# VIS4ROB-lab/covins

Hardware: AMD Instinct MI355X
Metric: GBA iterations/sec, 5-agent EuRoC merged map (higher is better)
Workload: dtype f64

## Files before the change

### covins_amd/csrc/common.hpp

```cpp
#pragma once
#include <hip/hip_runtime.h>
#include <atomic>
#include <cstdlib>
#include <stdint.h>

#include <map>
#include <unordered_map>
#include <utility>
#include <vector>

#include "../../include/covgpu.h"

namespace covgpu {

constexpr int kTile = 128;

struct DevProblem {
  int K, A, L, O, I, E, S;
  int D;
  int n;
  int npad;
  int N;
  int vi;
  int lm_group;
// ... 26 lines not shown
  double *pre_delta;
  double *pre_J;
  double *pre_P;
  double *pre_W;
  double *pre_bias;

  int *edge_i, *edge_j;
  double *edge_meas, *edge_sqrt_info, *edge_loss_a;

  int nchains;
  int max_chain_len;
  int* perm;
  int* pos_kf;
  int* chain_ptr;
  int* pos_chain_end;

  double* Sred;
  double* bred;
  double *Ad, *Ae;
  double *Bp, *Bs, *Bn;
  int* pos_chain_begin;
  double* bp;
  double* grad;
  double* hdiag;
  double* HllInv;
  double* gn;
  double* step;
  double* vtmp;
  double* Linv;
  double* scal;
  double* part;
  int part_n, part_imu, part_edge, part_vec;
  double *imuAd, *imuBs, *imuCd, *imuG;
  double* edgeOut;
  int *kf_edge_ptr, *kf_edge_ent;
  int nepairs;
  int *epair_ptr, *epair_i, *epair_j, *epair_ent;
  int* flag;

  int shard;
  double* vw;

  int nd, nd_nnodes, nd_nlev, nd_maxd;
  int *nd_vnode, *nd_voff, *nd_vord;
  int *nd_vown;
  int *nd_ndepth, *nd_nI;
  long long* nd_ntab;
  int* nd_abase;
  int* nd_fidx;
  double *nd_M, *nd_rhs, *nd_Linv;
  double* nd_dummy;

  double* tr;
  double* scal_r; int* flag_r;

  int uni;
  int* cam_model;
  double* cam_xi;
};

enum {
  TR_RADIUS = 0, TR_MU, TR_LMDF, TR_COST, TR_ALPHA, TR_GG, TR_GN2, TR_GDOT, TR_DNORM, TR_CG, TR_CN, TR_MODEL, TR_SN, TR_RHO, TR_COSTNEW,
  TR_OK, TR_VALID, TR_ACC, TR_TERM, TR_FNCONV, TR_RETRY, TR_FIRST, TR_INITCOST, TR_REUSE,
  TR_JA, TR_JB, TR_JC, TR_VV, TR_VG, TR_NN, TR_XN2,
  TR_COUNT = 32
};
// ... 396 lines not shown
```

### covins_amd/csrc/k_inertial.hip

```cpp
#include "common.hpp"
#include "dev_math.hpp"
#include "reduce.hpp"
#include "inertial_dev.hpp"

namespace covgpu {
using namespace covdev;

__global__ __launch_bounds__(64 * kImuWaves) void k_preintegrate(DevProblem P) {
  __shared__ double sm[kImuWaves][225 * 4 + 270];
  const int lane = threadIdx.x & 63, wave = threadIdx.x >> 6;
  const int f = blockIdx.x * kImuWaves + wave;
  const bool live = f < P.I;
  double* F = sm[wave];
  double* J = F + 225;
  double* C = J + 225;
  double* T = C + 225;
  double* V = T + 225;
  const int fj = live ? P.imu_j[f] : 0;
  const V3 ba = ld3(P.sb + 9 * fj + 3), bg = ld3(P.sb + 9 * fj + 6);
  for (int k = lane; k < 225; k += 64) { F[k] = 0.0; J[k] = (k % 16 == 0) ? 1.0 : 0.0; C[k] = 0.0; }
  for (int k = lane; k < 270; k += 64) V[k] = 0.0;
  V3 dp = v3(0, 0, 0), dv = v3(0, 0, 0);
  Q4 dq = Q4{0, 0, 0, 1};
  double dtsum = 0.0;
  V3 a0 = live ? ld3(P.imu_first + 6 * (size_t)f) : v3(0, 0, 0), w0 = live ? ld3(P.imu_first + 6 * (size_t)f + 3) : v3(0, 0, 0);
  const double* nz = P.imu_noise + 5 * (size_t)(live ? f : 0);
  const double sa = nz[0], sg = nz[1], saw = nz[2], sgw = nz[3];
  const double nd[6] = {sa * sa, sg * sg, sa * sa, sg * sg, saw * saw, sgw * sgw};
  const M3 I3 = ident3();
  __shared__ int s_steps[kImuWaves];
  if (lane == 0) s_steps[wave] = live ? P.imu_ptr[f + 1] - P.imu_ptr[f] : 0;
  __syncthreads();
  int nmax = 0;
#pragma unroll
  for (int k = 0; k < kImuWaves; ++k) nmax = max(nmax, s_steps[k]);
  const int s0 = live ? P.imu_ptr[f] : 0, ns = s_steps[wave];
  for (int it = 0; it < nmax; ++it) {
    const bool on = it < ns;
    if (on && lane == 0) {
      const double* smp = P.imu_samples + 7 * (size_t)(s0 + it);
      const double dt = smp[0];
      const V3 a1 = ld3(smp + 1), w1 = ld3(smp + 4);
      const V3 w = (w0 + w1) * 0.5 - bg;
      const Q4 dq1 = qnormalize(qmul(dq, Q4{w.x * dt * 0.5, w.y * dt * 0.5, w.z * dt * 0.5, 1.0}));
      const M3 Rq = qrot(dq), Rr = qrot(dq1);
      const V3 abar = (mul(Rq, a0 - ba) + mul(Rr, a1 - ba)) * 0.5;
      const V3 dp1 = dp + dv * dt + abar * (0.5 * dt * dt);
      const V3 dv1 = dv + abar * dt;
      const M3 RqA0 = mul(Rq, skew(a0 - ba)), RrA1 = mul(Rr, skew(a1 - ba));
      const M3 ImO = add(I3, scaled(skew(w), -dt));
      const M3 RrA1ImO = mul(RrA1, ImO);
      const M3 RqRr = add(Rq, Rr);
      const double dt2 = dt * dt, dt3 = dt2 * dt;
      set3(F, 15, 0, 0, I3, 1.0);
      set3(F, 15, 0, 3, add(scaled(RqA0, -0.25 * dt2), scaled(RrA1ImO, -0.25 * dt2)), 1.0);
      set3(F, 15, 0, 6, I3, dt);
      set3(F, 15, 0, 9, RqRr, -0.25 * dt2);
      set3(F, 15, 0, 12, RrA1, 0.25 * dt3);
      set3(F, 15, 3, 3, ImO, 1.0);
      set3(F, 15, 3, 12, I3, -dt);
      set3(F, 15, 6, 3, add(scaled(RqA0, -0.5 * dt), scaled(RrA1ImO, -0.5 * dt)), 1.0);
      set3(F, 15, 6, 6, I3, 1.0);
      set3(F, 15, 6, 9, RqRr, -0.5 * dt);
      set3(F, 15, 6, 12, RrA1, 0.5 * dt2);
      set3(F, 15, 9, 9, I3, 1.0);
      set3(F, 15, 12, 12, I3, 1.0);
      set3(V, 18, 0, 0, Rq, 0.25 * dt2);
      set3(V, 18, 0, 3, RrA1, -0.125 * dt3);
      set3(V, 18, 0, 6, Rr, 0.25 * dt2);
      set3(V, 18, 0, 9, RrA1, -0.125 * dt3);
      set3(V, 18, 3, 3, I3, 0.5 * dt);
      set3(V, 18, 3, 9, I3, 0.5 * dt);
      set3(V, 18, 6, 0, Rq, 0.5 * dt);
      set3(V, 18, 6, 3, RrA1, -0.25 * dt2);
      set3(V, 18, 6, 6, Rr, 0.5 * dt);
      set3(V, 18, 6, 9, RrA1, -0.25 * dt2);
      set3(V, 18, 9, 12, I3, dt);
      set3(V, 18, 12, 15, I3, dt);
      dp = dp1; dv = dv1; dq = dq1; dtsum += dt;
      a0 = a1; w0 = w1;
    }
    __syncthreads();
    double jn[4], tn[4];
    if (on) {
#pragma unroll
      for (int u = 0; u < 4; ++u) {
        const int e = lane + 64 * u;
        if (e < 225) {
          const int r = e / 15, c = e - 15 * r;
          double s2 = 0.0, s3 = 0.0;
#pragma unroll
          for (int k = 0; k < 15; ++k) { s2 += F[15 * r + k] * J[15 * k + c]; s3 += F[15 * r + k] * C[15 * k + c]; }
          jn[u] = s2; tn[u] = s3;
        }
      }
    }
    __syncthreads();
    if (on) {
#pragma unroll
      for (int u = 0; u < 4; ++u) {
        const int e = lane + 64 * u;
        if (e < 225) { J[e] = jn[u]; T[e] = tn[u]; }
      }
    }
    __syncthreads();
    if (on) {
#pragma unroll
      for (int u = 0; u < 4; ++u) {
        const int e = lane + 64 * u;
        if (e < 225) {
          const int r = e / 15, c = e - 15 * r;
          double s2 = 0.0;
#pragma unroll
          for (int k = 0; k < 15; ++k) s2 += T[15 * r + k] * F[15 * c + k];
#pragma unroll
          for (int k = 0; k < 18; ++k) s2 += V[18 * r + k] * nd[k / 3] * V[18 * c + k];
          C[e] = s2;
        }
      }
    }
    __syncthreads();
  }
  if (!live) return;
  if (lane == 0) {
    double* d = P.pre_delta + 11 * (size_t)f;
    d[0] = dp.x; d[1] = dp.y; d[2] = dp.z; d[3] = dq.x; d[4] = dq.y; d[5] = dq.z; d[6] = dq.w;
    d[7] = dv.x; d[8] = dv.y; d[9] = dv.z; d[10] = dtsum;
    double* pb = P.pre_bias + 6 * (size_t)f;
    pb[0] = ba.x; pb[1] = ba.y; pb[2] = ba.z; pb[3] = bg.x; pb[4] = bg.y; pb[5] = bg.z;
  }
  for (int k = lane; k < 225; k += 64) { P.pre_J[225 * (size_t)f + k] = J[k]; P.pre_P[225 * (size_t)f + k] = C[k]; }
  __builtin_amdgcn_fence(__ATOMIC_ACQ_REL, "workgroup");
  __builtin_amdgcn_wave_barrier();
  double* Wm = P.pre_W + 225 * (size_t)f;
  if (lane == 0) {
    bool ok = true;
    for (int c = 0; c < 15 && ok; ++c) {
      double dd = C[16 * c];
      for (int k = 0; k < c; ++k) dd -= C[15 * c + k] * C[15 * c + k];
      if (!(dd > 0.0)) { ok = false; break; }
      dd = sqrt(dd);
      C[16 * c] = dd;
      for (int r = c + 1; r < 15; ++r) {
        double s2 = C[15 * r + c];
        for (int k = 0; k < c; ++k) s2 -= C[15 * r + k] * C[15 * c + k];
        C[15 * r + c] = s2 / dd;
      }
    }
    for (int k = 0; k < 225; ++k) F[k] = 0.0;
    if (!ok) atomicAdd(P.flag + 1, 1);
    if (ok)
      for (int c = 0; c < 15; ++c) {
        F[16 * c] = 1.0 / C[16 * c];
        for (int r = c + 1; r < 15; ++r) {
          double s2 = 0.0;
          for (int k = c; k < r; ++k) s2 += C[15 * r + k] * F[15 * k + c];
          F[15 * r + c] = -s2 / C[16 * r];
        }
      }
    for (int k = 0; k < 225; ++k) Wm[k] = F[k];
  }
}

__global__ __launch_bounds__(64 * kImuWaves) void k_imu_build(DevProblem P) {
  __shared__ double sm[kImuWaves][kImuLds];
  const int lane = threadIdx.x & 63, wave = threadIdx.x >> 6;
  const int f = blockIdx.x * kImuWaves + wave;
  const bool live = f < P.I;
  double* sl = sm[wave];
  imu_stage<true>(P, P.pose, P.sb, f, live, lane, sl);
  {
    double c2 = (live && lane < 15) ? 0.5 * sl[1141 + lane] * sl[1141 + lane] : 0.0;
    c2 = wave_sum(c2);
    part_put(P, SC_COST, P.part_imu + blockIdx.x * kImuWaves + wave, c2);
  }
  if (!live) return;
  const double* Jw = sl + 450;
  const double* r = sl + 1141;
  const int i = P.imu_i[f], j = P.imu_j[f];
  const int pi = P.perm[i], pj = P.perm[j];
  const size_t K = (size_t)P.K;
  if (lane < 30) {
    const int a = lane, role = a / 15, la = a % 15;
    double ga = 0.0, haa = 0.0;
    for (int k = 0; k < 15; ++k) { ga += Jw[30 * k + a] * r[k]; haa += Jw[30 * k + a] * Jw[30 * k + a]; }
    double* g = P.imuG + (role * K + (role ? pj : pi)) * 30;
    g[la] = ga; g[15 + la] = haa;
  }
  for (int e = lane; e < 900; e += 64) {
    const int a = e / 30, b = e - 30 * a;
    const int ga_ = a / 15, la = a % 15, gb_ = b / 15, lb = b % 15;
    double h = 0.0;
#pragma unroll
    for (int k = 0; k < 15; ++k) h += Jw[30 * k + a] * Jw[30 * k + b];
    const size_t slot = ga_ * K + (ga_ ? pj : pi);
    if (la < 6 && lb < 6) {
      if (ga_ == gb_) P.imuCd[slot * 36 + 6 * la + lb] = h;
      else if (ga_ == 1) P.imuCd[(2 * K + pj) * 36 + 6 * la + lb] = h;
    } else if (la >= 6 && lb >= 6) {
      if (ga_ == gb_) P.imuAd[slot * 81 + 9 * (la - 6) + (lb - 6)] = h;
      else if (ga_ == 1) P.Ae[(size_t)81 * pj + 9 * (la - 6) + (lb - 6)] = h;
    } else if (la >= 6) {
      if (ga_ == gb_) P.imuBs[slot * 54 + 6 * (la - 6) + lb] = h;
      else if (ga_ == 0) P.Bn[(size_t)54 * pi + 6 * (la - 6) + lb] = h;
      else P.Bp[(size_t)54 * pj + 6 * (la - 6) + lb] = h;
    }
  }
}

__global__ __launch_bounds__(256) void k_imu_gather(DevProblem P, int which) {
  const int t = blockIdx.x * blockDim.x + threadIdx.x;
// ... 99 lines not shown
```

### covins_amd/csrc/k_tail.hip

```cpp
#include "between_dev.hpp"
#include "common.hpp"
#include "dev_math.hpp"
#include "inertial_dev.hpp"
#include "reduce.hpp"
#include "visual_dev.hpp"

namespace covgpu {
using namespace covdev;

static inline int tail_grid(int n, int cap) {
  const int b = (n + 255) / 256;
  return b < 1 ? 1 : (b > cap ? cap : b);
}
COV_DEV void tail_put(const DevProblem& P, double v, int slot, int index) {
  v = wave_sum(v);
  part_put(P, slot, index, v);
}

__global__ __launch_bounds__(256) void k_tail_stats(DevProblem P) {
  double gg = 0, gn2 = 0, gd = 0, gm = 0, vv = 0, vg = 0, nn = 0, xn = 0;
  const int stride = gridDim.x * blockDim.x, t0 = blockIdx.x * blockDim.x + threadIdx.x;
  for (int q = t0; q < P.N; q += stride) {
    const double g = P.grad[q], d = clamp_diag(P.hdiag[q]), s = P.gn[q];
    const double w = P.vw ? P.vw[q] : 1.0;
    const double c = g / (d * d);
    P.vtmp[q] = c;
    gg += w * (g / d) * (g / d); gn2 += w * (d * s) * (d * s); gd += w * g * s; gm = fmax(gm, w * fabs(g));
    vv += w * c * c; vg += w * c * s; nn += w * s * s;
  }
  for (int t = t0; t < P.K; t += stride) {
    const double wp = P.vw ? P.vw[(size_t)P.D * t] : 1.0, ws = (P.vw && P.vi) ? P.vw[(size_t)P.D * t + 6] : 1.0;
    if (!P.fixed[t]) for (int k = 0; k < 7; ++k) xn += wp * P.pose[7 * t + k] * P.pose[7 * t + k];
    if (P.vi) for (int k = 0; k < 9; ++k) xn += ws * P.sb[9 * t + k] * P.sb[9 * t + k];
  }
  for (int q = t0; q < 3 * P.L; q += stride) xn += P.lm[q] * P.lm[q];
  const int idx = P.part_vec + blockIdx.x * 4 + (threadIdx.x >> 6);
  tail_put(P, gg, SC_GG, idx); tail_put(P, gn2, SC_GN2, idx); tail_put(P, gd, SC_GDOT, idx);
  tail_put(P, vv, SC_VV, idx); tail_put(P, vg, SC_VG, idx); tail_put(P, nn, SC_NN, idx); tail_put(P, xn, SC_XN2, idx);
#pragma unroll
  for (int off = 32; off >= 1; off >>= 1) gm = fmax(gm, __shfl_xor(gm, off, 64));
  if ((threadIdx.x & 63) == 0) atomicMax(reinterpret_cast<unsigned long long*>(&P.scal[SC_GMAX]), (unsigned long long)__double_as_longlong(gm));
}

static_assert(kImuWaves == 4, "k_tail_jvp / k_tail_cost index their IMU and edge segments as 4 waves / 256 threads per workgroup");
template <bool TWO, bool UNI>
__global__ __launch_bounds__(64 * kImuWaves) void k_tail_jvp(DevProblem P, const double* __restrict__ va, const double* __restrict__ vb, int nb_obs, int nb_imu) {
  __shared__ double sm[kImuWaves][kImuLds];
  const int lane = threadIdx.x & 63, wave = threadIdx.x >> 6;
  double ja = 0.0, jb = 0.0, jc = 0.0;
  int idx;
  if ((int)blockIdx.x < nb_obs) {
    for (int o = blockIdx.x * blockDim.x + threadIdx.x; o < P.O; o += nb_obs * blockDim.x) {
      ObsLin e;
      const int kf = P.obs_kf[o], l = P.obs_lm[o];
      eval_obs<true, UNI>(P, P.pose, P.lm, o, kf, l, e);
      {
        const double* vp = vb + (size_t)P.D * kf;
        const double* vl = vb + P.n + 3 * (size_t)l;
        double s0 = e.jl[0] * vl[0] + e.jl[1] * vl[1] + e.jl[2] * vl[2];
        double s1 = e.jl[3] * vl[0] + e.jl[4] * vl[1] + e.jl[5] * vl[2];
#pragma unroll
        for (int k = 0; k < 6; ++k) { s0 += e.jp[k] * vp[k]; s1 += e.jp[6 + k] * vp[k]; }
        jb += s0 * s0 + s1 * s1;
        if (TWO) {
          const double* up = va + (size_t)P.D * kf;
          const double* ul = va + P.n + 3 * (size_t)l;
          double t0 = e.jl[0] * ul[0] + e.jl[1] * ul[1] + e.jl[2] * ul[2];
          double t1 = e.jl[3] * ul[0] + e.jl[4] * ul[1] + e.jl[5] * ul[2];
#pragma unroll
          for (int k = 0; k < 6; ++k) { t0 += e.jp[k] * up[k]; t1 += e.jp[6 + k] * up[k]; }
          ja += t0 * t0 + t1 * t1; jc += t0 * s0 + t1 * s1;
        }
      }
    }
    idx = blockIdx.x * 4 + wave;
  } else if ((int)blockIdx.x < nb_obs + nb_imu) {
    const int bi = blockIdx.x - nb_obs;
    const int f = bi * kImuWaves + wave;
    const bool live = f < P.I;
    double* sl = sm[wave];
    imu_stage<true>(P, P.pose, P.sb, f, live, lane, sl);
    if (live && lane < 15) {
      const double* Jw = sl + 450;
      const size_t oi = 15 * (size_t)P.imu_i[f], oj = 15 * (size_t)P.imu_j[f];
      double s2 = 0.0, t2 = 0.0;
      for (int c = 0; c < 15; ++c) {
        s2 += Jw[30 * lane + c] * vb[oi + c] + Jw[30 * lane + 15 + c] * vb[oj + c];
        if (TWO) t2 += Jw[30 * lane + c] * va[oi + c] + Jw[30 * lane + 15 + c] * va[oj + c];
      }
      jb = s2 * s2; ja = t2 * t2; jc = s2 * t2;
    }
    idx = P.part_imu + bi * kImuWaves + wave;
  } else {
    const int be = blockIdx.x - nb_obs - nb_imu;
    const int e = be * 256 + threadIdx.x;
    if (e < P.E) {
      double r[6], J[72];
      eval_edge<true>(P, P.pose, e, r, J);
      const size_t oi = (size_t)P.D * P.edge_i[e], oj = (size_t)P.D * P.edge_j[e];
#pragma unroll
      for (int a = 0; a < 6; ++a) {
        double s = 0.0, t = 0.0;
#pragma unroll
        for (int c = 0; c < 6; ++c) {
          s += J[12 * a + c] * vb[oi + c] + J[12 * a + 6 + c] * vb[oj + c];
          if (TWO) t += J[12 * a + c] * va[oi + c] + J[12 * a + 6 + c] * va[oj + c];
        }
        jb += s * s; ja += t * t; jc += s * t;
      }
    }
    idx = P.part_edge + be * 4 + wave;
    if (be * 4 + wave >= (P.E + 63) / 64) idx = -1;
  }
  jb = wave_sum(jb);
  if (TWO) { ja = wave_sum(ja); jc = wave_sum(jc); }
  if (idx >= 0) {
    part_put(P, SC_JB, idx, jb);
    if (TWO) { part_put(P, SC_JA, idx, ja); part_put(P, SC_JC, idx, jc); }
  }
}

template <bool UNI>
// ... 143 lines not shown
  if (stage == 1) tail_logic_a(P, tc, fresh, rd, P.flag_r[0]);
  else tail_logic_b(P, tc, rd);
}

__global__ __launch_bounds__(256) void k_tail_apply(DevProblem P) {
  const double cg = P.tr[TR_CG], cn = P.tr[TR_CN];
  const int t = blockIdx.x * blockDim.x + threadIdx.x;
  auto st = [&](size_t q) { const double s = cn * P.gn[q]; return cg != 0.0 ? s + cg * P.vtmp[q] : s; };
  if (t < P.K) {
    const size_t b = (size_t)P.D * t;
    const double* x = P.pose + 7 * t;
    double* y = P.pose_c + 7 * t;
    if (P.fixed[t]) {
      for (int k = 0; k < 7; ++k) y[k] = x[k];
    } else {
      const Q4 q = qnormalize(qmul(ldq(x), qexp(V3{st(b), st(b + 1), st(b + 2)})));
      y[0] = q.x; y[1] = q.y; y[2] = q.z; y[3] = q.w;
      y[4] = x[4] + st(b + 3); y[5] = x[5] + st(b + 4); y[6] = x[6] + st(b + 5);
    }
    if (P.vi)
      for (int k = 0; k < 9; ++k) P.sb_c[9 * t + k] = P.sb[9 * t + k] + st(b + 6 + k);
  }
  for (int q = t; q < 3 * P.L; q += gridDim.x * blockDim.x) P.lm_c[q] = P.lm[q] + st((size_t)P.n + q);
}

static inline void tail_segments(const DevProblem& P, int& nb_obs, int& nb_imu, int& nb_edge) {
  nb_obs = P.O > 0 ? tail_grid(P.O, 2048) : 0;
  nb_imu = (P.vi && P.I > 0) ? (P.I + kImuWaves - 1) / kImuWaves : 0;
  nb_edge = P.E > 0 ? (P.E + 255) / 256 : 0;
}
void launch_tail_stats(const DevProblem& P, hipStream_t st) {
  hipLaunchKernelGGL(k_tail_stats, dim3(tail_grid(P.N, 256)), dim3(256), 0, st, P);
}
void launch_tail_jvp(const DevProblem& P, bool two, hipStream_t st) {
  int a, b, c;
  tail_segments(P, a, b, c);
  if (a + b + c == 0) return;
  if (P.uni) {
    if (two) hipLaunchKernelGGL((k_tail_jvp<true, true>), dim3(a + b + c), dim3(64 * kImuWaves), 0, st, P, (const double*)P.vtmp, (const double*)P.gn, a, b);
    else hipLaunchKernelGGL((k_tail_jvp<false, true>), dim3(a + b + c), dim3(64 * kImuWaves), 0, st, P, (const double*)nullptr, (const double*)P.gn, a, b);
    return;
  }
  if (two) hipLaunchKernelGGL((k_tail_jvp<true, false>), dim3(a + b + c), dim3(64 * kImuWaves), 0, st, P, (const double*)P.vtmp, (const double*)P.gn, a, b);
  else hipLaunchKernelGGL((k_tail_jvp<false, false>), dim3(a + b + c), dim3(64 * kImuWaves), 0, st, P, (const double*)nullptr, (const double*)P.gn, a, b);
}
void launch_tail_cost(const DevProblem& P, hipStream_t st) {
  int a, b, c;
  tail_segments(P, a, b, c);
  if (a + b + c == 0) return;
  if (P.uni) hipLaunchKernelGGL(k_tail_cost<true>, dim3(a + b + c), dim3(64 * kImuWaves), 0, st, P, a, b);
  else hipLaunchKernelGGL(k_tail_cost<false>, dim3(a + b + c), dim3(64 * kImuWaves), 0, st, P, a, b);
}
void launch_tail_finish(const DevProblem& P, TrConsts tc, int stage, bool two, bool with_logic, int fresh, hipStream_t st) {
  SlotList sl;
  sl.n = 0;
  auto add = [&](int s) { sl.slot[sl.n++] = s; };
  if (stage == 1) {
    add(SC_GG); add(SC_GN2); add(SC_GDOT); add(SC_VV); add(SC_VG); add(SC_NN); add(SC_XN2); add(SC_JB);
    if (two) { add(SC_JA); add(SC_JC); }
  } else add(SC_COST);
  for (int i = sl.n; i < 12; ++i) sl.slot[i] = 0;
  hipLaunchKernelGGL(k_tail_finish, dim3(sl.n), dim3(1024), 0, st, P, sl, tc, with_logic ? stage : 0, fresh);
}
void launch_tail_logic(const DevProblem& P, TrConsts tc, int stage, int fresh, hipStream_t st) {
  hipLaunchKernelGGL(k_tail_logic, dim3(1), dim3(64), 0, st, P, tc, stage, fresh);
}
void launch_tail_apply(const DevProblem& P, hipStream_t st) {
  const int n = P.K > 3 * P.L ? P.K : 3 * P.L;
  int g = (P.K + 255) / 256;
  const int g2 = tail_grid(n, 2048);
  if (g2 > g) g = g2;
  hipLaunchKernelGGL(k_tail_apply, dim3(g), dim3(256), 0, st, P);
}

}
```

### covins_amd/csrc/solver.hip

```cpp
#include <dlfcn.h>

#include <algorithm>
#include <atomic>
#include <chrono>
#include <condition_variable>
#include <memory>
#include <mutex>
#include <cmath>
#include <cstdio>
#include <cstdlib>
#include <cstring>
#include <string>
#include <thread>
#include <vector>

#include "common.hpp"
#include "nd_plan.hpp"

using namespace covgpu;

static thread_local std::string g_err;
extern "C" const char* covgpu_last_error(void) { return g_err.c_str(); }

#define HIPCHK(expr)                                                                            \
// ... 812 lines not shown
  RC(dev_upload(c, &P.edge_i, (const int*)p->edge_i, (size_t)P.E));
  RC(dev_upload(c, &P.edge_j, (const int*)p->edge_j, (size_t)P.E));
  RC(dev_upload(c, &P.edge_meas, p->edge_meas, (size_t)7 * P.E));
  RC(dev_upload(c, &P.edge_sqrt_info, p->edge_sqrt_info, (size_t)36 * P.E));
  RC(dev_upload(c, &P.edge_loss_a, p->edge_loss_a, (size_t)P.E));
  RC(dev_upload(c, &P.perm, perm.data(), K)); RC(dev_upload(c, &P.pos_kf, pos_kf.data(), K));
  RC(dev_upload(c, &P.chain_ptr, chain_ptr.data(), chain_ptr.size()));
  RC(dev_upload(c, &P.pos_chain_end, chain_end.data(), K));
  RC(dev_alloc(c, &P.bred, (size_t)P.n));
  RC(dev_alloc(c, &P.bp, (size_t)2 * P.npad));
  const size_t Kv = vi ? K : 0;
  RC(dev_alloc(c, &P.Ad, 81 * Kv)); RC(dev_alloc(c, &P.Ae, 81 * Kv));
  RC(dev_alloc(c, &P.Bp, 54 * Kv)); RC(dev_alloc(c, &P.Bs, 54 * Kv)); RC(dev_alloc(c, &P.Bn, 54 * Kv));
  {
    std::vector<int> cbeg(P.K);
    for (int ch = 0; ch < P.nchains; ++ch) for (int q = chain_ptr[ch]; q < chain_ptr[ch + 1]; ++q) cbeg[q] = chain_ptr[ch];
    RC(dev_upload(c, &P.pos_chain_begin, cbeg.data(), cbeg.size()));
    HIPCHK(hipStreamSynchronize(c->st));
  }
  RC(dev_alloc(c, &P.grad, (size_t)P.N)); RC(dev_alloc(c, &P.hdiag, (size_t)P.N));
  RC(dev_alloc(c, &P.HllInv, (size_t)6 * P.L));
  RC(dev_alloc(c, &P.gn, (size_t)P.N)); RC(dev_alloc(c, &P.step, (size_t)P.N)); RC(dev_alloc(c, &P.vtmp, (size_t)P.N));
  HIPCHK(hipMemsetAsync(P.gn, 0, (size_t)P.N * sizeof(double), c->st)); HIPCHK(hipMemsetAsync(P.step, 0, (size_t)P.N * sizeof(double), c->st));
  HIPCHK(hipMemsetAsync(P.vtmp, 0, (size_t)P.N * sizeof(double), c->st));
  RC(dev_alloc(c, &P.scal, (size_t)SC_COUNT)); RC(dev_alloc(c, &P.flag, (size_t)4));
  RC(dev_alloc(c, &P.tr, (size_t)TR_COUNT));
  P.scal_r = P.scal; P.flag_r = P.flag;
  P.part_imu = 8192; P.part_edge = P.part_imu + ((P.I + 3) / 4) * 4; P.part_vec = P.part_edge + (P.E + 63) / 64;
  P.part_n = P.part_vec + 8192;
  RC(dev_alloc(c, &P.part, (size_t)SC_COUNT * P.part_n));
  HIPCHK(hipMemsetAsync(P.part, 0, (size_t)SC_COUNT * P.part_n * sizeof(double), c->st));
  RC(dev_alloc(c, &P.imuAd, 2 * 81 * Kv)); RC(dev_alloc(c, &P.imuBs, 2 * 54 * Kv));
  RC(dev_alloc(c, &P.imuCd, 3 * 36 * Kv)); RC(dev_alloc(c, &P.imuG, 2 * 30 * Kv));
  RC(dev_alloc(c, &P.edgeOut, (size_t)132 * P.E));
  {
    std::vector<int> kptr(P.K + 1, 0), kent(2 * (size_t)P.E);
    for (int e = 0; e < P.E; ++e) {
      if (p->edge_i[e] == p->edge_j[e]) { g_err = "invalid problem: self edge"; return COVGPU_ERR_INVALID_ARG; }
      kptr[p->edge_i[e] + 1]++; kptr[p->edge_j[e] + 1]++;
    }
    for (int k = 0; k < P.K; ++k) kptr[k + 1] += kptr[k];
    { std::vector<int> cur(kptr.begin(), kptr.end() - 1);
      for (int e = 0; e < P.E; ++e) { kent[cur[p->edge_i[e]]++] = 2 * e; kent[cur[p->edge_j[e]]++] = 2 * e + 1; } }
    struct PE { int i, j, ent; };
    std::vector<PE> pe(P.E);
    for (int e = 0; e < P.E; ++e) {
      const int a = perm[p->edge_i[e]], b = perm[p->edge_j[e]];
      pe[e] = (a > b) ? PE{a, b, 2 * e} : PE{b, a, 2 * e + 1};
    }
    std::stable_sort(pe.begin(), pe.end(), [](const PE& x, const PE& y) { return x.i != y.i ? x.i < y.i : x.j < y.j; });
    std::vector<int> eptr, ei, ej, eent(P.E);
    for (int q = 0; q < P.E; ++q) {
      if (q == 0 || pe[q].i != pe[q - 1].i || pe[q].j != pe[q - 1].j) { eptr.push_back(q); ei.push_back(pe[q].i); ej.push_back(pe[q].j); }
      eent[q] = pe[q].ent;
    }
    eptr.push_back(P.E);
    P.nepairs = (int)ei.size();
    RC(dev_upload(c, &P.kf_edge_ptr, kptr.data(), kptr.size())); RC(dev_upload(c, &P.kf_edge_ent, kent.data(), kent.size()));
    RC(dev_upload(c, &P.epair_ptr, eptr.data(), eptr.size())); RC(dev_upload(c, &P.epair_i, ei.data(), ei.size()));
    RC(dev_upload(c, &P.epair_j, ej.data(), ej.size())); RC(dev_upload(c, &P.epair_ent, eent.data(), eent.size()));
    HIPCHK(hipStreamSynchronize(c->st));
    tm("IMU, edges, vectors");
    if (use_nd) {
      NdHostPlan nhp;
      if (c->sharded) {
        if ((int)c->shard_plan->K != P.K || (c->shard_plan->vi != 0) != vi) { g_err = "sharded solve: the problem does not match the shard plan"; return COVGPU_ERR_INVALID_ARG; }
// ... 279 lines not shown
        if (why) { if (!c->coll_failed) { c->coll_failed = true; c->coll_err = why; } c->reducer->abort(); break; }
      } else if (spins > 256) std::this_thread::sleep_for(std::chrono::microseconds(50));
    }
  }
  HIPCHK(hipStreamSynchronize(c->st));
  HIPCHK(hipGetLastError());
  if (dist_sharded(c) && (c->coll_failed || c->chol.gate_failed())) return dist_fail(c);
  if (c->chol.gate_failed()) {
    g_err = "solve: a device-flag gate between the context's streams timed out (COVGPU_GATE_TIMEOUT_S; COVGPU_GATES=0 selects HIP events)";
    return COVGPU_ERR_GATE_TIMEOUT;
  }
  if (c->coll_failed) {
    if (c->reducer) c->reducer->abort();
    if (c->peer_fail) c->peer_fail->store(1);
    g_err = (c->sharded ? "sharded solve, rank " + std::to_string(c->rank) + ": " : std::string("solve: ")) + c->coll_err;
    return COVGPU_ERR_NO_DEVICE;
  }
  return COVGPU_OK;
}

static int solve_impl_dev(covgpu_context* c, const covgpu_options* opt, covgpu_result* res) {
  if (!c->have) { g_err = "no problem uploaded"; return COVGPU_ERR_INVALID_ARG; }
  HIPCHK(hipSetDevice(c->device));
  DevProblem& P = c->P;
  const covgpu_options& o = *opt;
  P.reproj_loss_a = o.reproj_loss_a;
  std::memset(res, 0, sizeof(*res));
  c->coll_failed = false; c->coll_err.clear();
  const auto t_begin = std::chrono::steady_clock::now();
  c->chol.init();
  if (c->sharded) c->chol.gate_timeout_s = std::max(c->chol.gate_timeout_s, 120.0);
  RC(reset_state(c));
  HIPCHK(hipMemsetAsync(P.flag + 1, 0, sizeof(int), c->st));
  launch_preintegrate(P, c->st);
  double* h = c->h_tr;
  std::memset(h, 0, TR_COUNT * sizeof(double));
  h[TR_RADIUS] = o.initial_radius; h[TR_MU] = 1e-8; h[TR_LMDF] = 2.0; h[TR_FIRST] = 1.0; h[TR_OK] = 1.0;
  HIPCHK(hipMemcpyAsync(P.tr, h, TR_COUNT * sizeof(double), hipMemcpyHostToDevice, c->st));
  HIPCHK(hipStreamSynchronize(c->st));
  const TrConsts tc{o.strategy, o.max_radius, o.min_relative_decrease, o.function_tolerance, o.parameter_tolerance, o.gradient_tolerance};
  bool reuse = false, got_initial = false;
  int it = 0, accepted = 0, term = 0;
  static const bool fused_tail = env_int("COVGPU_TAIL", 1) != 0;
  const bool two = o.strategy == COVGPU_DOGLEG;
  const bool coll = c->sharded && c->reducer != nullptr;
  bool use_box = false;
  while (it < o.max_iterations) {
    use_box = false;
    if (fused_tail) {
      if (!reuse) {
        const double damp = (o.strategy == COVGPU_LM) ? 1.0 / h[TR_RADIUS] : h[TR_MU];
        enqueue_build(c, damp);
        enqueue_solve(c, P.gn);
        launch_tail_stats(P, c->st);
        launch_tail_jvp(P, two, c->st);
        launch_tail_finish(P, tc, 1, two, !coll, 1, c->st);
        if (coll) { reduce_scalars(c); launch_tail_logic(P, tc, 1, 1, c->st); }
      } else launch_tail_logic(P, tc, 1, 0, c->st);
      launch_tail_apply(P, c->st);
      launch_tail_cost(P, c->st);
      launch_tail_finish(P, tc, 2, two, !coll, 0, c->st);
      if (coll) { reduce_scalars(c); launch_tail_logic(P, tc, 2, 0, c->st); }
      static const bool dev_aids = getenv("COVGPU_TRACE_PANELS") != nullptr || getenv("COVGPU_GATE_LOG") != nullptr;
      use_box = c->d_box != nullptr && !coll && !c->profiling && !dev_aids;
      if (use_box) c->box_seq += 1.0;
      launch_tr_accept(P, c->st, use_box ? c->d_box : nullptr, c->box_seq);
    } else {
    if (!reuse) {
      const double damp = (o.strategy == COVGPU_LM) ? 1.0 / h[TR_RADIUS] : h[TR_MU];
      enqueue_build(c, damp);
      enqueue_solve(c, P.gn);
      if (o.strategy == COVGPU_DOGLEG) { launch_cauchy_vec(P, c->st); enqueue_jvp(c, P.vtmp); }
// ... 1314 lines not shown
```

Before: 291.2.

## Cache IMU whitened Jacobians for tail JVP and restructure preintegration kernel

The IMU build kernel now stores each factor's whitened Jacobian in a new device buffer (imuJw). The tail JVP kernel reads that buffer instead of re-running imu_stage every iteration; the old path stays behind the COVGPU_IMU_JW env switch. Preintegration is rewritten to exploit the sparsity of F and V with compact 11- and 12-column layouts, to use wave-level syncs instead of block-wide ones, to prefetch the next IMU sample, and to run the Cholesky and inverse across lanes instead of lane 0 alone. Preintegration is also launched on a different stream (chol.mid) after the host sync, which relies on some ordering against the later build kernels that is not visible here. The cache costs extra memory traffic and 450 doubles of storage per factor.

Result: faster. 297.5 (median of 6 runs) (+2.2%).

```diff
diff --git a/covins_amd/csrc/common.hpp b/covins_amd/csrc/common.hpp
--- a/covins_amd/csrc/common.hpp
+++ b/covins_amd/csrc/common.hpp
@@ -82,6 +82,7 @@
   double* part;
   int part_n, part_imu, part_edge, part_vec;
   double *imuAd, *imuBs, *imuCd, *imuG;
+  double* imuJw;
   double* edgeOut;
   int *kf_edge_ptr, *kf_edge_ent;
   int nepairs;
diff --git a/covins_amd/csrc/k_inertial.hip b/covins_amd/csrc/k_inertial.hip
--- a/covins_amd/csrc/k_inertial.hip
+++ b/covins_amd/csrc/k_inertial.hip
@@ -6,122 +6,162 @@
 namespace covgpu {
 using namespace covdev;
 
+COV_DEV void wave_sync() {
+  __builtin_amdgcn_fence(__ATOMIC_ACQ_REL, "workgroup");
+  __builtin_amdgcn_wave_barrier();
+}
+COV_DEV int f_col(int r, int t) {
+  if (r < 3) return t == 0 ? r : t < 4 ? 2 + t : t == 4 ? 6 + r : 4 + t;
+  if (r < 6) return t < 3 ? 3 + t : t == 3 ? 9 + r : 0;
+  if (r < 9) return t < 3 ? 3 + t : t == 3 ? r : t < 10 ? 5 + t : 0;
+  return t == 0 ? r : 0;
+}
+COV_DEV unsigned long long f_cols(int r) {
+  unsigned long long p = 0;
+#pragma unroll
+  for (int t = 0; t < 11; ++t) p |= (unsigned long long)f_col(r, t) << (4 * t);
+  return p;
+}
+constexpr int kPreLds = 225 + 225 + 135 + 165 + 108 + 1;
+static_assert(135 + 165 >= 225, "the whitening matrix is inverted in the slice of T and Fs");
+
 __global__ __launch_bounds__(64 * kImuWaves) void k_preintegrate(DevProblem P) {
-  __shared__ double sm[kImuWaves][225 * 4 + 270];
-  const int lane = threadIdx.x & 63, wave = threadIdx.x >> 6;
-  const int f = blockIdx.x * kImuWaves + wave;
-  const bool live = f < P.I;
-  double* F = sm[wave];
-  double* J = F + 225;
+  __shared__ double sm[kImuWaves][kPreLds];
+  const int lane = threadIdx.x & 63, wave = threadIdx.x >> 6;
+  const int f = blockIdx.x * kImuWaves + wave;
+  if (f >= P.I) return;
+  double* J = sm[wave];
   double* C = J + 225;
   double* T = C + 225;
-  double* V = T + 225;
-  const int fj = live ? P.imu_j[f] : 0;
+  double* Fs = T + 135;
+  double* Vs = Fs + 165;
+  double* sdt = Vs + 108;
+  const int fj = P.imu_j[f];
   const V3 ba = ld3(P.sb + 9 * fj + 3), bg = ld3(P.sb + 9 * fj + 6);
-  for (int k = lane; k < 225; k += 64) { F[k] = 0.0; J[k] = (k % 16 == 0) ? 1.0 : 0.0; C[k] = 0.0; }
-  for (int k = lane; k < 270; k += 64) V[k] = 0.0;
+  for (int k = lane; k < 225; k += 64) { J[k] = (k % 16 == 0) ? 1.0 : 0.0; C[k] = 0.0; }
+  for (int k = lane; k < 165; k += 64) {
+    const int r = k / 11, t = k - 11 * r;
+    Fs[k] = ((r < 3 || r >= 9) ? t == 0 : (r >= 6 && t == 3)) ? 1.0 : 0.0;
+  }
+  for (int k = lane; k < 108; k += 64) Vs[k] = 0.0;
   V3 dp = v3(0, 0, 0), dv = v3(0, 0, 0);
   Q4 dq = Q4{0, 0, 0, 1};
   double dtsum = 0.0;
-  V3 a0 = live ? ld3(P.imu_first + 6 * (size_t)f) : v3(0, 0, 0), w0 = live ? ld3(P.imu_first + 6 * (size_t)f + 3) : v3(0, 0, 0);
-  const double* nz = P.imu_noise + 5 * (size_t)(live ? f : 0);
+  V3 a0 = ld3(P.imu_first + 6 * (size_t)f), w0 = ld3(P.imu_first + 6 * (size_t)f + 3);
+  const double* nz = P.imu_noise + 5 * (size_t)f;
   const double sa = nz[0], sg = nz[1], saw = nz[2], sgw = nz[3];
   const double nd[6] = {sa * sa, sg * sg, sa * sa, sg * sg, saw * saw, sgw * sgw};
   const M3 I3 = ident3();
-  __shared__ int s_steps[kImuWaves];
-  if (lane == 0) s_steps[wave] = live ? P.imu_ptr[f + 1] - P.imu_ptr[f] : 0;
-  __syncthreads();
-  int nmax = 0;
-#pragma unroll
-  for (int k = 0; k < kImuWaves; ++k) nmax = max(nmax, s_steps[k]);
-  const int s0 = live ? P.imu_ptr[f] : 0, ns = s_steps[wave];
-  for (int it = 0; it < nmax; ++it) {
-    const bool on = it < ns;
-    if (on && lane == 0) {
-      const double* smp = P.imu_samples + 7 * (size_t)(s0 + it);
+  const int s0 = P.imu_ptr[f], ns = P.imu_ptr[f + 1] - s0;
+  M3 Rq = qrot(dq), RqA0 = mul(Rq, skew(a0 - ba));
+  V3 Rqa0 = mul(Rq, a0 - ba);
+  unsigned long long pr[3], pc[4];
+#pragma unroll
+  for (int u = 0; u < 3; ++u) pr[u] = f_cols(min((lane + 64 * u) / 15, 14));
+#pragma unroll
+  for (int u = 0; u < 4; ++u) pc[u] = f_cols(min(lane + 64 * u, 224) % 15);
+  double smp[7];
+  if (lane == 0 && ns > 0) {
+#pragma unroll
+    for (int k = 0; k < 7; ++k) smp[k] = P.imu_samples[7 * (size_t)s0 + k];
+  }
+  wave_sync();
+  for (int it = 0; it < ns; ++it) {
+    if (lane == 0) {
       const double dt = smp[0];
-      const V3 a1 = ld3(smp + 1), w1 = ld3(smp + 4);
+      const V3 a1 = v3(smp[1], smp[2], smp[3]), w1 = v3(smp[4], smp[5], smp[6]);
+      if (it + 1 < ns) {
+#pragma unroll
+        for (int k = 0; k < 7; ++k) smp[k] = P.imu_samples[7 * (size_t)(s0 + it + 1) + k];
+      }
       const V3 w = (w0 + w1) * 0.5 - bg;
       const Q4 dq1 = qnormalize(qmul(dq, Q4{w.x * dt * 0.5, w.y * dt * 0.5, w.z * dt * 0.5, 1.0}));
-      const M3 Rq = qrot(dq), Rr = qrot(dq1);
-      const V3 abar = (mul(Rq, a0 - ba) + mul(Rr, a1 - ba)) * 0.5;
+      const M3 Rr = qrot(dq1);
+      const V3 Rra1 = mul(Rr, a1 - ba);
+      const V3 abar = (Rqa0 + Rra1) * 0.5;
       const V3 dp1 = dp + dv * dt + abar * (0.5 * dt * dt);
       const V3 dv1 = dv + abar * dt;
-      const M3 RqA0 = mul(Rq, skew(a0 - ba)), RrA1 = mul(Rr, skew(a1 - ba));
+      const M3 RrA1 = mul(Rr, skew(a1 - ba));
       const M3 ImO = add(I3, scaled(skew(w), -dt));
       const M3 RrA1ImO = mul(RrA1, ImO);
       const M3 RqRr = add(Rq, Rr);
       const double dt2 = dt * dt, dt3 = dt2 * dt;
-      set3(F, 15, 0, 0, I3, 1.0);
-      set3(F, 15, 0, 3, add(scaled(RqA0, -0.25 * dt2), scaled(RrA1ImO, -0.25 * dt2)), 1.0);
-      set3(F, 15, 0, 6, I3, dt);
-      set3(F, 15, 0, 9, RqRr, -0.25 * dt2);
-      set3(F, 15, 0, 12, RrA1, 0.25 * dt3);
-      set3(F, 15, 3, 3, ImO, 1.0);
-      set3(F, 15, 3, 12, I3, -dt);
-      set3(F, 15, 6, 3, add(scaled(RqA0, -0.5 * dt), scaled(RrA1ImO, -0.5 * dt)), 1.0);
-      set3(F, 15, 6, 6, I3, 1.0);
-      set3(F, 15, 6, 9, RqRr, -0.5 * dt);
-      set3(F, 15, 6, 12, RrA1, 0.5 * dt2);
-      set3(F, 15, 9, 9, I3, 1.0);
-      set3(F, 15, 12, 12, I3, 1.0);
-      set3(V, 18, 0, 0, Rq, 0.25 * dt2);
-      set3(V, 18, 0, 3, RrA1, -0.125 * dt3);
-      set3(V, 18, 0, 6, Rr, 0.25 * dt2);
-      set3(V, 18, 0, 9, RrA1, -0.125 * dt3);
-      set3(V, 18, 3, 3, I3, 0.5 * dt);
-      set3(V, 18, 3, 9, I3, 0.5 * dt);
-      set3(V, 18, 6, 0, Rq, 0.5 * dt);
-      set3(V, 18, 6, 3, RrA1, -0.25 * dt2);
-      set3(V, 18, 6, 6, Rr, 0.5 * dt);
-      set3(V, 18, 6, 9, RrA1, -0.25 * dt2);
-      set3(V, 18, 9, 12, I3, dt);
-      set3(V, 18, 12, 15, I3, dt);
+      set3(Fs, 11, 0, 1, add(scaled(RqA0, -0.25 * dt2), scaled(RrA1ImO, -0.25 * dt2)), 1.0);
+      set3(Fs, 11, 0, 5, RqRr, -0.25 * dt2);
+      set3(Fs, 11, 0, 8, RrA1, 0.25 * dt3);
+      set3(Fs, 11, 3, 0, ImO, 1.0);
+      set3(Fs, 11, 6, 0, add(scaled(RqA0, -0.5 * dt), scaled(RrA1ImO, -0.5 * dt)), 1.0);
+      set3(Fs, 11, 6, 4, RqRr, -0.5 * dt);
+      set3(Fs, 11, 6, 7, RrA1, 0.5 * dt2);
+      set3(Vs, 12, 0, 0, Rq, 0.25 * dt2);
+      set3(Vs, 12, 0, 3, RrA1, -0.125 * dt3);
+      set3(Vs, 12, 0, 6, Rr, 0.25 * dt2);
+      set3(Vs, 12, 0, 9, RrA1, -0.125 * dt3);
+      set3(Vs, 12, 6, 0, Rq, 0.5 * dt);
+      set3(Vs, 12, 6, 3, RrA1, -0.25 * dt2);
+      set3(Vs, 12, 6, 6, Rr, 0.5 * dt);
+      set3(Vs, 12, 6, 9, RrA1, -0.25 * dt2);
+#pragma unroll
+      for (int i = 0; i < 3; ++i) {
+        Fs[11 * i + 4] = dt;
+        Fs[11 * (3 + i) + 3] = -dt;
+        Vs[12 * (3 + i) + 3 + i] = 0.5 * dt;
+        Vs[12 * (3 + i) + 9 + i] = 0.5 * dt;
+      }
+      sdt[0] = dt;
       dp = dp1; dv = dv1; dq = dq1; dtsum += dt;
       a0 = a1; w0 = w1;
-    }
-    __syncthreads();
-    double jn[4], tn[4];
-    if (on) {
-#pragma unroll
-      for (int u = 0; u < 4; ++u) {
-        const int e = lane + 64 * u;
-        if (e < 225) {
-          const int r = e / 15, c = e - 15 * r;
-          double s2 = 0.0, s3 = 0.0;
-#pragma unroll
-          for (int k = 0; k < 15; ++k) { s2 += F[15 * r + k] * J[15 * k + c]; s3 += F[15 * r + k] * C[15 * k + c]; }
-          jn[u] = s2; tn[u] = s3;
+      Rq = Rr; RqA0 = RrA1; Rqa0 = Rra1;
+    }
+    wave_sync();
+    double jn[3];
+#pragma unroll
+    for (int u = 0; u < 3; ++u) {
+      const int e = lane + 64 * u;
+      if (e < 135) {
+        const int r = e / 15, c = e - 15 * r;
+        double s2 = 0.0, s3 = 0.0;
+#pragma unroll
+        for (int t = 0; t < 11; ++t) {
+          const int k = (int)(pr[u] >> (4 * t)) & 15;
+          const double fv = Fs[11 * r + t];
+          s2 = fma(fv, J[15 * k + c], s2);
+          s3 = fma(fv, C[15 * k + c], s3);
         }
+        jn[u] = s2; T[e] = s3;
       }
     }
-    __syncthreads();
-    if (on) {
-#pragma unroll
-      for (int u = 0; u < 4; ++u) {
-        const int e = lane + 64 * u;
-        if (e < 225) { J[e] = jn[u]; T[e] = tn[u]; }
+    wave_sync();
+    const double dt = sdt[0];
+    double cn[4];
+#pragma unroll
+    for (int u = 0; u < 4; ++u) {
+      const int e = lane + 64 * u;
+      if (u < 3 && e < 135) J[e] = jn[u];
+      if (e < 225) {
+        const int r = e / 15, c = e - 15 * r;
+        const double* Tr = r < 9 ? T + 15 * r : C + 15 * r;
+        double s2 = 0.0;
+#pragma unroll
+        for (int t = 0; t < 11; ++t) {
+          const int k = (int)(pc[u] >> (4 * t)) & 15;
+          s2 = fma(Tr[k], Fs[11 * c + t], s2);
+        }
+        if (r < 9 && c < 9) {
+#pragma unroll
+          for (int k = 0; k < 12; ++k) s2 = fma(Vs[12 * r + k] * nd[k / 3], Vs[12 * c + k], s2);
+        } else if (r == c) s2 = fma(dt * (r < 12 ? nd[4] : nd[5]), dt, s2);
+        cn[u] = s2;
       }
     }
-    __syncthreads();
-    if (on) {
-#pragma unroll
-      for (int u = 0; u < 4; ++u) {
-        const int e = lane + 64 * u;
-        if (e < 225) {
-          const int r = e / 15, c = e - 15 * r;
-          double s2 = 0.0;
-#pragma unroll
-          for (int k = 0; k < 15; ++k) s2 += T[15 * r + k] * F[15 * c + k];
-#pragma unroll
-          for (int k = 0; k < 18; ++k) s2 += V[18 * r + k] * nd[k / 3] * V[18 * c + k];
-          C[e] = s2;
-        }
-      }
-    }
-    __syncthreads();
-  }
-  if (!live) return;
+    wave_sync();
+#pragma unroll
+    for (int u = 0; u < 4; ++u) {
+      const int e = lane + 64 * u;
+      if (e < 225) C[e] = cn[u];
+    }
+    wave_sync();
+  }
   if (lane == 0) {
     double* d = P.pre_delta + 11 * (size_t)f;
     d[0] = dp.x; d[1] = dp.y; d[2] = dp.z; d[3] = dq.x; d[4] = dq.y; d[5] = dq.z; d[6] = dq.w;
@@ -130,36 +170,36 @@
     pb[0] = ba.x; pb[1] = ba.y; pb[2] = ba.z; pb[3] = bg.x; pb[4] = bg.y; pb[5] = bg.z;
   }
   for (int k = lane; k < 225; k += 64) { P.pre_J[225 * (size_t)f + k] = J[k]; P.pre_P[225 * (size_t)f + k] = C[k]; }
-  __builtin_amdgcn_fence(__ATOMIC_ACQ_REL, "workgroup");
-  __builtin_amdgcn_wave_barrier();
-  double* Wm = P.pre_W + 225 * (size_t)f;
-  if (lane == 0) {
-    bool ok = true;
-    for (int c = 0; c < 15 && ok; ++c) {
-      double dd = C[16 * c];
-      for (int k = 0; k < c; ++k) dd -= C[15 * c + k] * C[15 * c + k];
-      if (!(dd > 0.0)) { ok = false; break; }
-      dd = sqrt(dd);
-      C[16 * c] = dd;
-      for (int r = c + 1; r < 15; ++r) {
-        double s2 = C[15 * r + c];
-        for (int k = 0; k < c; ++k) s2 -= C[15 * r + k] * C[15 * c + k];
-        C[15 * r + c] = s2 / dd;
-      }
-    }
-    for (int k = 0; k < 225; ++k) F[k] = 0.0;
-    if (!ok) atomicAdd(P.flag + 1, 1);
-    if (ok)
-      for (int c = 0; c < 15; ++c) {
-        F[16 * c] = 1.0 / C[16 * c];
-        for (int r = c + 1; r < 15; ++r) {
-          double s2 = 0.0;
-          for (int k = c; k < r; ++k) s2 += C[15 * r + k] * F[15 * k + c];
-          F[15 * r + c] = -s2 / C[16 * r];
-        }
-      }
-    for (int k = 0; k < 225; ++k) Wm[k] = F[k];
-  }
+  double* Wi = T;
+  for (int k = lane; k < 225; k += 64) Wi[k] = 0.0;
+  wave_sync();
+  bool ok = true;
+  for (int c = 0; c < 15; ++c) {
+    double dd = C[16 * c];
+    for (int k = 0; k < c; ++k) dd -= C[15 * c + k] * C[15 * c + k];
+    if (!(dd > 0.0)) { ok = false; break; }
+    dd = sqrt(dd);
+    const int r = c + 1 + lane;
+    if (r < 15) {
+      double s2 = C[15 * r + c];
+      for (int k = 0; k < c; ++k) s2 -= C[15 * r + k] * C[15 * c + k];
+      C[15 * r + c] = s2 / dd;
+    }
+    if (lane == 0) C[16 * c] = dd;
+    wave_sync();
+  }
+  if (!ok && lane == 0) atomicAdd(P.flag + 1, 1);
+  if (ok && lane < 15) {
+    const int c = lane;
+    Wi[16 * c] = 1.0 / C[16 * c];
+    for (int r = c + 1; r < 15; ++r) {
+      double s2 = 0.0;
+      for (int k = c; k < r; ++k) s2 += C[15 * r + k] * Wi[15 * k + c];
+      Wi[15 * r + c] = -s2 / C[16 * r];
+    }
+  }
+  wave_sync();
+  for (int k = lane; k < 225; k += 64) P.pre_W[225 * (size_t)f + k] = Wi[k];
 }
 
 __global__ __launch_bounds__(64 * kImuWaves) void k_imu_build(DevProblem P) {
@@ -177,6 +217,7 @@
   if (!live) return;
   const double* Jw = sl + 450;
   const double* r = sl + 1141;
+  for (int k = lane; k < 450; k += 64) P.imuJw[450 * (size_t)f + k] = Jw[k];
   const int i = P.imu_i[f], j = P.imu_j[f];
   const int pi = P.perm[i], pj = P.perm[j];
   const size_t K = (size_t)P.K;
diff --git a/covins_amd/csrc/k_tail.hip b/covins_amd/csrc/k_tail.hip
--- a/covins_amd/csrc/k_tail.hip
+++ b/covins_amd/csrc/k_tail.hip
@@ -43,9 +43,16 @@
 }
 
 static_assert(kImuWaves == 4, "k_tail_jvp / k_tail_cost index their IMU and edge segments as 4 waves / 256 threads per workgroup");
-template <bool TWO, bool UNI>
+template <bool TWO>
+COV_DEV void imu_row_jvp(const double* Jw, int row, const double* __restrict__ va, const double* __restrict__ vb, size_t oi, size_t oj, double& s2, double& t2) {
+  s2 = 0.0; t2 = 0.0;
+  for (int c = 0; c < 15; ++c) {
+    s2 += Jw[30 * row + c] * vb[oi + c] + Jw[30 * row + 15 + c] * vb[oj + c];
+    if (TWO) t2 += Jw[30 * row + c] * va[oi + c] + Jw[30 * row + 15 + c] * va[oj + c];
+  }
+}
+template <bool TWO, bool UNI, bool JW>
 __global__ __launch_bounds__(64 * kImuWaves) void k_tail_jvp(DevProblem P, const double* __restrict__ va, const double* __restrict__ vb, int nb_obs, int nb_imu) {
-  __shared__ double sm[kImuWaves][kImuLds];
   const int lane = threadIdx.x & 63, wave = threadIdx.x >> 6;
   double ja = 0.0, jb = 0.0, jc = 0.0;
   int idx;
@@ -78,16 +85,17 @@
     const int bi = blockIdx.x - nb_obs;
     const int f = bi * kImuWaves + wave;
     const bool live = f < P.I;
-    double* sl = sm[wave];
-    imu_stage<true>(P, P.pose, P.sb, f, live, lane, sl);
+    const double* Jw = P.imuJw + 450 * (size_t)(live ? f : 0);
+    if constexpr (!JW) {
+      __shared__ double sm[kImuWaves][kImuLds];
+      double* sl = sm[wave];
+      imu_stage<true>(P, P.pose, P.sb, f, live, lane, sl);
+      Jw = sl + 450;
+    }
     if (live && lane < 15) {
-      const double* Jw = sl + 450;
       const size_t oi = 15 * (size_t)P.imu_i[f], oj = 15 * (size_t)P.imu_j[f];
-      double s2 = 0.0, t2 = 0.0;
-      for (int c = 0; c < 15; ++c) {
-        s2 += Jw[30 * lane + c] * vb[oi + c] + Jw[30 * lane + 15 + c] * vb[oj + c];
-        if (TWO) t2 += Jw[30 * lane + c] * va[oi + c] + Jw[30 * lane + 15 + c] * va[oj + c];
-      }
+      double s2, t2;
+      imu_row_jvp<TWO>(Jw, lane, va, vb, oi, oj, s2, t2);
       jb = s2 * s2; ja = t2 * t2; jc = s2 * t2;
     }
     idx = P.part_imu + bi * kImuWaves + wave;
@@ -297,17 +305,26 @@
 void launch_tail_stats(const DevProblem& P, hipStream_t st) {
   hipLaunchKernelGGL(k_tail_stats, dim3(tail_grid(P.N, 256)), dim3(256), 0, st, P);
 }
+template <bool TWO, bool UNI, bool JW>
+static void tail_jvp_go(const DevProblem& P, int nb, int a, int b, hipStream_t st) {
+  hipLaunchKernelGGL((k_tail_jvp<TWO, UNI, JW>), dim3(nb), dim3(64 * kImuWaves), 0, st, P, TWO ? (const double*)P.vtmp : (const double*)nullptr, (const double*)P.gn, a, b);
+}
 void launch_tail_jvp(const DevProblem& P, bool two, hipStream_t st) {
   int a, b, c;
   tail_segments(P, a, b, c);
   if (a + b + c == 0) return;
-  if (P.uni) {
-    if (two) hipLaunchKernelGGL((k_tail_jvp<true, true>), dim3(a + b + c), dim3(64 * kImuWaves), 0, st, P, (const double*)P.vtmp, (const double*)P.gn, a, b);
-    else hipLaunchKernelGGL((k_tail_jvp<false, true>), dim3(a + b + c), dim3(64 * kImuWaves), 0, st, P, (const double*)nullptr, (const double*)P.gn, a, b);
-    return;
-  }
-  if (two) hipLaunchKernelGGL((k_tail_jvp<true, false>), dim3(a + b + c), dim3(64 * kImuWaves), 0, st, P, (const double*)P.vtmp, (const double*)P.gn, a, b);
-  else hipLaunchKernelGGL((k_tail_jvp<false, false>), dim3(a + b + c), dim3(64 * kImuWaves), 0, st, P, (const double*)nullptr, (const double*)P.gn, a, b);
+  static const bool jw = env_int("COVGPU_IMU_JW", 1) != 0;
+  const int form = (two ? 4 : 0) | (P.uni ? 2 : 0) | (jw ? 1 : 0), nb = a + b + c;
+  switch (form) {
+    case 0: tail_jvp_go<false, false, false>(P, nb, a, b, st); break;
+    case 1: tail_jvp_go<false, false, true>(P, nb, a, b, st); break;
+    case 2: tail_jvp_go<false, true, false>(P, nb, a, b, st); break;
+    case 3: tail_jvp_go<false, true, true>(P, nb, a, b, st); break;
+    case 4: tail_jvp_go<true, false, false>(P, nb, a, b, st); break;
+    case 5: tail_jvp_go<true, false, true>(P, nb, a, b, st); break;
+    case 6: tail_jvp_go<true, true, false>(P, nb, a, b, st); break;
+    default: tail_jvp_go<true, true, true>(P, nb, a, b, st); break;
+  }
 }
 void launch_tail_cost(const DevProblem& P, hipStream_t st) {
   int a, b, c;
diff --git a/covins_amd/csrc/solver.hip b/covins_amd/csrc/solver.hip
--- a/covins_amd/csrc/solver.hip
+++ b/covins_amd/csrc/solver.hip
@@ -868,6 +868,7 @@
   HIPCHK(hipMemsetAsync(P.part, 0, (size_t)SC_COUNT * P.part_n * sizeof(double), c->st));
   RC(dev_alloc(c, &P.imuAd, 2 * 81 * Kv)); RC(dev_alloc(c, &P.imuBs, 2 * 54 * Kv));
   RC(dev_alloc(c, &P.imuCd, 3 * 36 * Kv)); RC(dev_alloc(c, &P.imuG, 2 * 30 * Kv));
+  RC(dev_alloc(c, &P.imuJw, (size_t)450 * P.I));
   RC(dev_alloc(c, &P.edgeOut, (size_t)132 * P.E));
   {
     std::vector<int> kptr(P.K + 1, 0), kent(2 * (size_t)P.E);
@@ -1213,12 +1214,12 @@
   if (c->sharded) c->chol.gate_timeout_s = std::max(c->chol.gate_timeout_s, 120.0);
   RC(reset_state(c));
   HIPCHK(hipMemsetAsync(P.flag + 1, 0, sizeof(int), c->st));
-  launch_preintegrate(P, c->st);
   double* h = c->h_tr;
   std::memset(h, 0, TR_COUNT * sizeof(double));
   h[TR_RADIUS] = o.initial_radius; h[TR_MU] = 1e-8; h[TR_LMDF] = 2.0; h[TR_FIRST] = 1.0; h[TR_OK] = 1.0;
   HIPCHK(hipMemcpyAsync(P.tr, h, TR_COUNT * sizeof(double), hipMemcpyHostToDevice, c->st));
   HIPCHK(hipStreamSynchronize(c->st));
+  launch_preintegrate(P, c->chol.mid);
   const TrConsts tc{o.strategy, o.max_radius, o.min_relative_decrease, o.function_tolerance, o.parameter_tolerance, o.gradient_tolerance};
   bool reuse = false, got_initial = false;
   int it = 0, accepted = 0, term = 0;
```
